# ZongyueQin/SessionSimilaritySearch

Hardware: AMD Instinct MI355X
Metric: session queries/sec (higher is better)
Workload: dtype f32

## Files before the change

### sessionsimilaritysearch_amd/csrc/scan.hip

```cpp
#include "scan_kernel.h"

namespace sss {

__device__ unsigned g_boot_expired;

extern "C" int sss_scan_boot_expired(int reset) {
    unsigned v = 0, zero = 0;
    if (hipMemcpyFromSymbol(&v, HIP_SYMBOL(g_boot_expired), sizeof(v)) != hipSuccess) { set_error("scan_boot_expired: read failed"); return SSS_EHIP; }
    if (reset && hipMemcpyToSymbol(HIP_SYMBOL(g_boot_expired), &zero, sizeof(zero)) != hipSuccess) { set_error("scan_boot_expired: reset failed"); return SSS_EHIP; }
    return (int)(v > 0x7fffffffu ? 0x7fffffffu : v);
}

int current_device() {
    int dev = 0;
    (void)hipGetDevice(&dev);
    return dev < 0 || dev >= MAX_DEVICES ? 0 : dev;
}

static int pick_splits(long n, int G, int tr) {
    int S = (256 / G) & ~7;
    if (S < 8) S = 8;
    while (S > 8 && (long)S * tr > n) S -= 8;
    return S;
}

constexpr int TR256_MIN_TILES = 24;

static size_t align256(size_t v) { return (v + 255) & ~(size_t)255; }

static ScanPlan make_plan_for(long nq, long n, int d, int k, int dtype, bool want_append);

static bool append_form_fits() {
    static int cached[MAX_DEVICES] = {};
    const int dev = current_device();
    if (cached[dev] == 0) {
        constexpr int lds = 2 * 128 * 256 + 8 * 2048;
        const void* fn = reinterpret_cast<const void*>(&k_scan<256, 128, DT_F16, 8, false, true>);
        int blocks = 0, cus = 0;
        bool ok = hipFuncSetAttribute(fn, hipFuncAttributeMaxDynamicSharedMemorySize, lds) == hipSuccess &&
                  hipOccupancyMaxActiveBlocksPerMultiprocessor(&blocks, fn, 512, lds) == hipSuccess &&
                  hipDeviceGetAttribute(&cus, hipDeviceAttributeMultiprocessorCount, dev) == hipSuccess;
        (void)hipGetLastError();
        cached[dev] = (ok && blocks >= 2 && cus >= 256) ? 1 : 2;
    }
    return cached[dev] == 1;
}

ScanPlan make_plan(long nq, long n, int d, int k, int dtype) {
    const int rb = d * elem_bytes(dtype);
    if (rb == 256 && dtype != DT_F32 && k <= KP && append_form_fits()) {
        const ScanPlan a = make_plan_for(nq, n, d, k, dtype, true);
        if (a.append) return a;
    }
    return make_plan_for(nq, n, d, k, dtype, false);
}
static ScanPlan make_plan_for(long nq, long n, int d, int k, int dtype, bool want_append) {
    ScanPlan p;
    const int rb = d * elem_bytes(dtype);
    const int wgq = rb == 1024 ? 128 : WG_QUERIES;
    p.G = (int)((nq + wgq - 1) / wgq);
    int tr = rb <= 512 ? 128 : 64;
    int S = pick_splits(n, p.G, tr);
    if (rb == 512 && (n + (long)S * 128 - 1) / ((long)S * 128) < 48) { tr = 64; S = pick_splits(n, p.G, tr); }
    if (rb == 256 && dtype != DT_F32 && n / ((long)S * 256) >= TR256_MIN_TILES) tr = 256;
    if (want_append) {
        tr = 128;
        S = pick_splits(n, p.G, tr);
        if ((long)S * p.G > 256 || (long)2 * S * tr * 7 > n) want_append = false;
        else S *= 2;
        if (!want_append) { ScanPlan none; none.append = 0; return none; }
    }
    p.tile_rows = tr;
    p.S = S;
    p.L = 2 * S;
    p.K2 = k + 2 <= KP ? (k + 2 < 8 ? 8 : k + 2) : k <= KP ? KP : k + 12;
    if ((long)p.L * KP < p.K2) p.K2 = p.L * KP;
    p.total_tiles = (int)((n + tr - 1) / tr);
    p.tiles_per_split = (p.total_tiles + S - 1) / S;
    p.cap = p.L * KP;
    const int active_splits = (p.total_tiles + p.tiles_per_split - 1) / p.tiles_per_split;
    p.J = p.K2 <= 128 ? 16 : 64;
    p.cert = 1;
    while (p.J * p.cert < p.K2 && p.cert < KP) p.cert *= 2;
    p.Ju = p.J;
    p.tau_skip = (p.cert == 1 && p.J == 16) ? 16 - p.K2 : 0;
    bool classes_ok = 2 * active_splits >= p.Ju;
    if (p.cert == 1 && p.J == 16 && active_splits < 16) {
        const int zero0 = active_splits < 8 ? 8 - active_splits : 0, zero1 = active_splits < 8 ? 8 : 16 - active_splits;
        classes_ok = zero0 <= (p.tau_skip >> 1) + (p.tau_skip & 1) && zero1 <= (p.tau_skip >> 1);
    }
    if (p.J * p.cert < p.K2 || !classes_ok) { p.J = 0; p.Ju = 0; p.tau_skip = 0; }
    p.boot = (p.J > 0 && p.cert == 1) ? 1 : 0;
    p.append = (want_append && p.boot) ? 1 : 0;
    if (want_append && !p.append) return p;
    if (p.append) p.cap = 2048;
    p.total_bytes = align256((size_t)nq * p.cap * 8);
    return p;
}

ScanPlan make_thr_plan(long nsel, long n, int d, int scan_dtype, int cap) {
    ScanPlan p = {};
    const int rb = d * elem_bytes(scan_dtype);
    const int wgq = rb == 1024 ? 128 : WG_QUERIES;
    p.G = (int)((nsel + wgq - 1) / wgq);
    p.tile_rows = rb <= 512 ? 128 : 64;
    p.S = pick_splits(n, p.G, p.tile_rows);
    p.L = 2 * p.S;
    p.total_tiles = (int)((n + p.tile_rows - 1) / p.tile_rows);
    p.tiles_per_split = (p.total_tiles + p.S - 1) / p.S;
    p.cap = cap;
    p.total_bytes = align256((size_t)nsel * cap * 8);
    return p;
}

int launch_scan(int dtype, int d, int tile_rows, const ScanArgs& a, hipStream_t st) {
    const int rb = d * elem_bytes(dtype);
    if (a.bias != nullptr) return launch_scan_l2(dtype, d, tile_rows, a, st);
    int rc = 1;
    with_dtype<true>(dtype, [&](auto dt) {
        constexpr int DT = decltype(dt)::value;
        rc = launch_shape<DT, 0>(rb, tile_rows, a, st);
    });
    if (rc != 1) return rc;
    set_error("scan: unsupported row size %d bytes", rb);
    return SSS_EINVAL;
}

}
```

### sessionsimilaritysearch_amd/csrc/scan_kernel.h

```cpp
#pragma once
#include "scan.h"
#include "scan_dev.h"

#ifndef SSS_STAGGER
#define SSS_STAGGER 1
#endif
#ifndef SSS_F32_SCHED
#define SSS_F32_SCHED 7
#endif

namespace sss {

extern __device__ unsigned g_boot_expired;

template <int RB, int TR, int DT, int NW, bool THR = false, bool AP = false, int MET = 0>
__global__ __launch_bounds__(NW * 64, AP ? 2 * (NW / 4) : NW / 4) void k_scan(const ScanArgs A) {
    constexpr int H = TR / 64;
    constexpr int CH = RB / 16;
    constexpr int NU = RB / 32;
    constexpr int TILE_BYTES = TR * RB;
    constexpr int LOADS_PER_WAVE = TR * CH / 64 / NW;
    constexpr int WGQ = NW * 32;
    constexpr bool PRECOMP = RB <= 512 && !AP;
    constexpr int TAU_LDS = 2 * TILE_BYTES;
    constexpr bool F32S = (SSS_F32_SCHED & 1) && DT == DT_F32 && !AP && !THR && RB == 512;
    static_assert(CH <= 64, "row longer than one LDS-DMA instruction");
    static_assert(LOADS_PER_WAVE >= 1, "a tile is at least one DMA piece per wave");
    extern __shared__ __attribute__((aligned(16))) char smem[];

    const int nq = A.nq, n = A.n, S = A.S, G = A.G, J = A.J;
    const char* __restrict__ Qb = reinterpret_cast<const char*>(A.Q);
    const char* __restrict__ Cb = reinterpret_cast<const char*>(A.C);
    const int tid = threadIdx.x;
    const int lane = tid & 63;
    const int wave = __builtin_amdgcn_readfirstlane(tid >> 6);
    const int r = lane & 31, h = lane >> 5;

    const int bid = blockIdx.x;
    const int xcd = bid & 7, slot = bid >> 3;
    const int split = xcd * (S >> 3) + slot / G;
    const int g = slot % G;

    const int q_local = wave * 32 + r;
    const int q_glob = g * WGQ + q_local;
    int q_ld = q_glob < nq ? q_glob : nq - 1;
    if constexpr (THR) q_ld = A.qsel[q_ld];
    f32x4 qc[NU];

    float ls[KP];
    int li[KP];
#pragma unroll
    for (int i = 0; i < KP; ++i) { ls[i] = -INFINITY; li[i] = -1; }
    float pend_s = -INFINITY;
    int pend_i = -1;
    constexpr int E = 4;
    float es[E];
    int ei[E];
    int ecnt = 0;
#pragma unroll
    for (int i = 0; i < E; ++i) { es[i] = -INFINITY; ei[i] = -1; }
    float tau = -INFINITY, thr = -INFINITY;
    if constexpr (THR) thr = q_glob < nq ? A.thr[q_glob] : INFINITY;
    float rmax = -INFINITY;
    float pub = -INFINITY;

    int tile_lo = split * A.tiles_per_split;
    int tile_hi = tile_lo + A.tiles_per_split;
    if (tile_hi > A.total_tiles) tile_hi = A.total_tiles;
    const int ntiles = tile_lo < tile_hi ? tile_hi - tile_lo : 0;
    const bool use_tau = !THR && J > 0;
    const bool boot = use_tau && A.boot && ntiles > 0;
    const int nb = boot ? 1 : 0;
    const int niter = ntiles + nb;
    auto tile_of = [&](int i) { return i < ntiles ? tile_lo + i : tile_lo; };
    const int skip = A.tau_skip;

    bool slots_seen = false;
    const unsigned* my_half = nullptr;
    unsigned cls_live = 0;
#ifdef SSS_EXP_NOPAIR
    const bool pair_pub = false;
#else
    const bool pair_pub = A.cert == 1;
#endif
    if (use_tau) {
        cls_live = pair_pub ? (unsigned)(split + (split >> 4)) & 15u : (unsigned)(2 * split + h) % (unsigned)A.Ju;
        my_half = A.slots + (size_t)q_ld * SLOT_STRIDE + h * (J >> 1);
    }
    auto tau_ord = [&]() -> unsigned {
        if (J == 16 && skip > 0) {
            unsigned v[8];
            load8_sc1(my_half, v);
            return tau_select16(v, skip, h);
        }
        unsigned m = 0xFFFFFFFFu;
        for (int v = 0; v < (J >> 1); v += 8) m = min(m, min8_sc1(my_half + v));
        return min(m, (unsigned)__shfl_xor((int)m, 32));
    };
    const unsigned tau_lds = (unsigned)(unsigned long)(lptr_c)smem + TAU_LDS + wave * 2048;
    auto tau_fetch = [&]() {
        int ln = lane;
        asm volatile("" : "+v"(ln));
#pragma unroll
        for (int j = 0; j < 2; ++j) {
            int qi = g * WGQ + wave * 32 + 16 * j + (ln >> 2);
            if (qi > nq - 1) qi = nq - 1;
            const unsigned off = (unsigned)qi * (unsigned)(SLOT_STRIDE * 4) + (unsigned)(ln & 3) * 16u;
            const unsigned dst = __builtin_amdgcn_readfirstlane(tau_lds + j * 1024);
            asm volatile("s_mov_b32 m0, %1\n\ts_nop 0\n\tglobal_load_lds_dwordx4 %0, %2 sc1"
                         : : "v"(off), "s"(dst), "s"(A.slots) : "memory");
        }
    };
    auto tau_read = [&]() -> unsigned {
        const u32x4* p = reinterpret_cast<const u32x4*>(smem + TAU_LDS + wave * 2048 + r * 64 + h * 32);
        const u32x4 a = p[0], b = p[1];
        if (skip > 0) {
            unsigned v[8] = {a.x, a.y, a.z, a.w, b.x, b.y, b.z, b.w};
            return tau_select16(v, skip, h);
        }
        const unsigned m = min(min(min(a.x, a.y), min(a.z, a.w)), min(min(b.x, b.y), min(b.z, b.w)));
        return min(m, (unsigned)__shfl_xor((int)m, 32));
    };
    auto set_tau = [&](unsigned m) {
        if (m > ORD_NEG_INF) tau = fmaxf(tau, ord2f(m - 1));
        thr = AP ? tau : fmaxf(ls[KP - 1], tau);
    };
    auto publish = [&](unsigned cls) {
        float val = rmax;
        bool ok = true;
        if (A.cert > 1) {
            float v2 = ls[1], v4 = ls[3], v8 = ls[7], v16 = ls[KP - 1];
            int i2 = li[1], i4 = li[3], i8 = li[7], i16 = li[KP - 1];
            asm volatile("" : "+v"(v2), "+v"(v4), "+v"(v8), "+v"(v16), "+v"(i2), "+v"(i4), "+v"(i8), "+v"(i16));
            const int c = A.cert;
            val = c == 2 ? v2 : c == 4 ? v4 : c == 8 ? v8 : v16;
            ok = (c == 2 ? i2 : c == 4 ? i4 : c == 8 ? i8 : i16) >= 0;
        }
        if (pair_pub) { val = fmaxf(val, __shfl_xor(val, 32)); ok = h == 0; }
        unsigned cur = 0u;
        if (J == 16 && slots_seen) cur = *reinterpret_cast<const unsigned*>(smem + TAU_LDS + wave * 2048 + r * 64 + cls * 4u);
        if (ok && val > pub && val > tau && f2ord(val) > cur && q_glob < nq) {
            int qq = THR ? q_ld : q_glob;
            asm volatile("" : "+v"(qq));
            __hip_atomic_fetch_max(A.slots + ((size_t)(unsigned)qq * (unsigned)SLOT_STRIDE + cls), f2ord(val), __ATOMIC_RELAXED, __HIP_MEMORY_SCOPE_AGENT);
            pub = val;
        }
    };

    const unsigned lds_base = (unsigned)(unsigned long)(lptr_c)smem;
    auto slot_row = [&](int i) { return ((wave * LOADS_PER_WAVE + i) * 64 + lane) / CH; };
    auto slot_off = [&](int i) {
        const int p = (wave * LOADS_PER_WAVE + i) * 64 + lane;
        const int tr = p / CH, sc = p % CH;
        return (unsigned)(tr * RB + ((sc ^ (tr & 15)) * 16));
    };
    unsigned lane_off[PRECOMP ? LOADS_PER_WAVE : 1];
    if (PRECOMP) {
#pragma unroll
        for (int i = 0; i < LOADS_PER_WAVE; ++i) lane_off[i] = slot_off(i);
    }
    auto stage_piece = [&](int buf, int tile_idx, int i) {
        const long row0 = (long)tile_idx * TR;
        const bool inside = row0 + TR <= (long)n;
        const char* tile_src = Cb + (size_t)row0 * RB;
        const unsigned dst = __builtin_amdgcn_readfirstlane(
            lds_base + buf * TILE_BYTES + (wave * LOADS_PER_WAVE + i) * 1024);
        unsigned off = PRECOMP ? lane_off[PRECOMP ? i : 0] : slot_off(i);
        if (!inside) {
            const int lr = slot_row(i);
            long grow = row0 + lr;
            if (grow > (long)n - 1) grow = (long)n - 1;
            off = (unsigned)((grow - row0) * RB) + (off - (unsigned)(lr * RB));
        }
        asm volatile("s_mov_b32 m0, %1\n\ts_nop 0\n\tglobal_load_lds_dwordx4 %0, %2"
                     : : "v"(off), "s"(dst), "s"(tile_src) : "memory");
    };
    auto stage = [&](int buf, int tile_idx) {
#pragma unroll
        for (int i = 0; i < LOADS_PER_WAVE; ++i) stage_piece(buf, tile_idx, i);
    };

    const int x = h ^ (r & 15);
    f32x16 acc0 = {0}, acc1 = {0};
    [[maybe_unused]] float bcur[MET ? 2 * H : 1];
    [[maybe_unused]] float bscale = 1.f;
    [[maybe_unused]] auto bias_fetch = [&](int tile_idx) {
#pragma unroll
        for (int s = 0; s < 2 * H; ++s) {
            long row = (long)tile_idx * TR + s * 32 + r;
            if (row > (long)n - 1) row = (long)n - 1;
            bcur[s] = h == 0 ? A.bias[row] : 0.f;
        }
    };
    [[maybe_unused]] auto bias_land = [&]() {
#pragma unroll
        for (int s = 0; s < 2 * H; ++s) asm volatile("" : "+v"(bcur[s]));
    };

    auto mfma_sub = [&](int buf, int sub, int next_tile) {
        const char* tile = smem + buf * TILE_BYTES + sub * (64 * RB);
        if constexpr (H == 1) { if (next_tile >= 0) stage(buf ^ 1, next_tile); }
        auto lda = [&](int u) -> const f32x4* {
            const int c = (2 * u) ^ x;
            return reinterpret_cast<const f32x4*>(tile + (r * CH + c) * 16);
        };
        constexpr int PF = DT == DT_F32 ? 1 : AP ? 1 : (RB == 256 ? NU : RB == 512 ? 4 : 2);
        f32x4 as0[NU], as1[NU];
#pragma unroll
        for (int u = 0; u < PF && u < NU; ++u) { const f32x4* p = lda(u); as0[u] = p[0]; as1[u] = p[32 * CH]; }
        const f32x16 zero = {0};
        if constexpr (MET) {
            float b0 = bcur[0], b1 = bcur[1];
#pragma unroll
            for (int s = 1; s < H; ++s) { b0 = sub == s ? bcur[2 * s] : b0; b1 = sub == s ? bcur[2 * s + 1] : b1; }
            acc0 = __builtin_amdgcn_mfma_f32_32x32x2f32(b0, bscale, zero, 0, 0, 0);
            acc1 = __builtin_amdgcn_mfma_f32_32x32x2f32(b1, bscale, zero, 0, 0, 0);
        } else {
            acc0 = zero; acc1 = zero;
        }
        [[maybe_unused]] i32x16 ia0 = {0}, ia1 = {0};
#pragma unroll
        for (int u = 0; u < NU; ++u) {
            if (u + PF < NU) { const f32x4* p = lda(u + PF); as0[u + PF] = p[0]; as1[u + PF] = p[32 * CH]; }
            const f32x4 a0 = as0[u], a1 = as1[u];
            __builtin_amdgcn_sched_barrier(0);
            if constexpr (DT == DT_F32) {
                acc0 = __builtin_amdgcn_mfma_f32_32x32x2f32(a0.x, qc[u].x, acc0, 0, 0, 0);
                acc1 = __builtin_amdgcn_mfma_f32_32x32x2f32(a1.x, qc[u].x, acc1, 0, 0, 0);
                acc0 = __builtin_amdgcn_mfma_f32_32x32x2f32(a0.y, qc[u].y, acc0, 0, 0, 0);
                acc1 = __builtin_amdgcn_mfma_f32_32x32x2f32(a1.y, qc[u].y, acc1, 0, 0, 0);
                acc0 = __builtin_amdgcn_mfma_f32_32x32x2f32(a0.z, qc[u].z, acc0, 0, 0, 0);
                acc1 = __builtin_amdgcn_mfma_f32_32x32x2f32(a1.z, qc[u].z, acc1, 0, 0, 0);
                acc0 = __builtin_amdgcn_mfma_f32_32x32x2f32(a0.w, qc[u].w, acc0, 0, 0, 0);
                acc1 = __builtin_amdgcn_mfma_f32_32x32x2f32(a1.w, qc[u].w, acc1, 0, 0, 0);
            } else if constexpr (DT == DT_BF16) {
                const bf16x8 qb = __builtin_bit_cast(bf16x8, qc[u]);
                acc0 = __builtin_amdgcn_mfma_f32_32x32x16_bf16(__builtin_bit_cast(bf16x8, a0), qb, acc0, 0, 0, 0);
                acc1 = __builtin_amdgcn_mfma_f32_32x32x16_bf16(__builtin_bit_cast(bf16x8, a1), qb, acc1, 0, 0, 0);
            } else if constexpr (DT == DT_F16 || DT == DT_H16) {
                const f16x8 qb = __builtin_bit_cast(f16x8, qc[u]);
                acc0 = __builtin_amdgcn_mfma_f32_32x32x16_f16(__builtin_bit_cast(f16x8, a0), qb, acc0, 0, 0, 0);
                acc1 = __builtin_amdgcn_mfma_f32_32x32x16_f16(__builtin_bit_cast(f16x8, a1), qb, acc1, 0, 0, 0);
            } else if constexpr (DT == DT_I8) {
                const i32x4 qb = __builtin_bit_cast(i32x4, qc[u]);
                ia0 = __builtin_amdgcn_mfma_i32_32x32x32_i8(__builtin_bit_cast(i32x4, a0), qb, ia0, 0, 0, 0);
                ia1 = __builtin_amdgcn_mfma_i32_32x32x32_i8(__builtin_bit_cast(i32x4, a1), qb, ia1, 0, 0, 0);
            } else {
                const bf16x8 A0 = __builtin_bit_cast(bf16x8, a0), A1 = __builtin_bit_cast(bf16x8, a1);
                const bf16x8 qh = __builtin_bit_cast(bf16x8, qc[u < NU / 2 ? u : u - NU / 2]);
                acc0 = __builtin_amdgcn_mfma_f32_32x32x16_bf16(A0, qh, acc0, 0, 0, 0);
                acc1 = __builtin_amdgcn_mfma_f32_32x32x16_bf16(A1, qh, acc1, 0, 0, 0);
                if (u < NU / 2) {
                    const bf16x8 ql = __builtin_bit_cast(bf16x8, qc[u + NU / 2]);
                    acc0 = __builtin_amdgcn_mfma_f32_32x32x16_bf16(A0, ql, acc0, 0, 0, 0);
                    acc1 = __builtin_amdgcn_mfma_f32_32x32x16_bf16(A1, ql, acc1, 0, 0, 0);
                }
            }
            __builtin_amdgcn_sched_barrier(0);
        }
        if constexpr (DT == DT_I8) {
            acc0 = __builtin_convertvector(ia0, f32x16);
            acc1 = __builtin_convertvector(ia1, f32x16);
        }
        if constexpr (H > 1) { if (sub == 0 && next_tile >= 0) stage(buf ^ 1, next_tile); }
    };

    auto block_max = [&](const f32x16& a, float& q0, float& q1, float& q2, float& q3) {
        q0 = fmaxf(fmaxf(a[0], a[1]), fmaxf(a[2], a[3]));
        q1 = fmaxf(fmaxf(a[4], a[5]), fmaxf(a[6], a[7]));
        q2 = fmaxf(fmaxf(a[8], a[9]), fmaxf(a[10], a[11]));
        q3 = fmaxf(fmaxf(a[12], a[13]), fmaxf(a[14], a[15]));
        return fmaxf(fmaxf(q0, q1), fmaxf(q2, q3));
    };
    auto insert_block = [&](const f32x16& a, int base) {
        float q0, q1, q2, q3;
        const float m = block_max(a, q0, q1, q2, q3);
        if (__builtin_amdgcn_ballot_w64(m > thr) == 0) return;
        auto walk = [&](float qm, int j0) {
            if (__builtin_amdgcn_ballot_w64(qm > thr) == 0) return;
#pragma unroll
            for (int jj = 0; jj < 4; ++jj) {
                const int j = j0 + jj;
                const bool pass = a[j] > thr;
                if (__builtin_amdgcn_ballot_w64(pass) != 0) {
                    if (__builtin_amdgcn_ballot_w64(pass && pend_i >= 0) != 0) {
                        list_insert<KP>(ls, li, pend_s, pend_i);
                        pend_s = -INFINITY; pend_i = -1;
                        thr = fmaxf(ls[KP - 1], tau);
                    }
                    const bool still = a[j] > thr;
                    pend_s = still ? a[j] : pend_s;
                    pend_i = still ? base + (j & 3) + 8 * (j >> 2) : pend_i;
                }
            }
        };
        walk(q0, 0); walk(q1, 4); walk(q2, 8); walk(q3, 12);
    };
    auto flush = [&](bool need) {
        if (need && q_glob < nq) {
            const unsigned at = atomicAdd(A.cnt + q_glob, (unsigned)ecnt);
            unsigned long long* dst = A.cand + (size_t)q_glob * A.cap;
            unsigned long long lost = 0ull;
#pragma unroll
            for (int i = 0; i < E; ++i) {
                if (i < ecnt) {
                    const unsigned long long key = make_key(es[i], ei[i]);
                    if (at + (unsigned)i < (unsigned)A.cap) dst[at + i] = key;
                    else lost = lost > key ? lost : key;
                }
            }
            if (lost != 0ull && A.maxlast != nullptr) atomicMax(A.maxlast + q_glob, lost);
        }
        ecnt = need ? 0 : ecnt;
    };
    auto append_block = [&](const f32x16& a, int base) {
        float q0, q1, q2, q3;
        const float m = block_max(a, q0, q1, q2, q3);
        if (__builtin_amdgcn_ballot_w64(m > thr) == 0) return;
        auto walk = [&](float qm, int j0) {
            if (__builtin_amdgcn_ballot_w64(qm > thr) == 0) return;
#pragma unroll
            for (int jj = 0; jj < 4; ++jj) {
                const int j = j0 + jj;
                const bool pass = a[j] > thr;
                if (__builtin_amdgcn_ballot_w64(pass) != 0) {
                    const bool full = pass && ecnt == E;
                    if (__builtin_amdgcn_ballot_w64(full) != 0) flush(full);
#pragma unroll
                    for (int i = E - 1; i > 0; --i) { es[i] = pass ? es[i - 1] : es[i]; ei[i] = pass ? ei[i - 1] : ei[i]; }
                    es[0] = pass ? a[j] : es[0];
                    ei[0] = pass ? base + (j & 3) + 8 * (j >> 2) : ei[0];
                    ecnt += pass ? 1 : 0;
                }
            }
        };
        walk(q0, 0); walk(q1, 4); walk(q2, 8); walk(q3, 12);
    };
    auto emit_block = [&](const f32x16& a, int base) {
        float q0, q1, q2, q3;
        const float m = block_max(a, q0, q1, q2, q3);
        if (__builtin_amdgcn_ballot_w64(m > thr) == 0) return;
#pragma unroll
        for (int j = 0; j < 16; ++j) {
            if (a[j] > thr) {
                const unsigned pos = atomicAdd(A.cnt + q_glob, 1u);
                if (pos < (unsigned)A.cap) A.cand[(size_t)q_glob * A.cap + pos] = make_key(a[j], base + (j & 3) + 8 * (j >> 2));
            }
        }
    };
    const bool two_ahead = H > 1 && niter > 1;
    if (ntiles > 0) stage(0, tile_lo);
    if (two_ahead) stage(1, tile_of(1));
    if constexpr (MET) {
        int q_shift = 0;
        load_queries<RB, DT>(Qb, q_ld, h, qc, &q_shift);
        if constexpr (DT == DT_F16) {
            const int e = A.corpus_shift + q_shift;
            bscale = ldexpf(1.f, e < -126 ? -126 : e > 127 ? 127 : e);
        }
        bias_fetch(tile_of(0));
    } else {
        load_queries<RB, DT>(Qb, q_ld, h, qc);
    }
    asm volatile("s_waitcnt vmcnt(0)" ::: "memory");
    __syncthreads();
    if constexpr (MET) bias_land();

    const int T = niter * H;
    long row0_of_step = 0;
    constexpr bool TAU_EVERY_TILE = TR >= 512;
    auto refresh_at = [&](int i) {
        if (i == 1 && boot && !TAU_EVERY_TILE) return false;
        if (TAU_EVERY_TILE || i <= 4) return true;
        const int sh = 30 - __builtin_clz(i);
        return (i & ((1 << sh) - 1)) == 0;
    };
    auto tile_top = [&](int i) {
        if (!use_tau || i == 0) return;
        if (J == 16) {
            if (!refresh_at(i)) return;
            publish(cls_live);
            tau_fetch();
            return;
        }
        const int ii = i - (wave >= 4 ? 1 : 0);
        if (ii >= 2 && (ii <= 8 || (ii & (ii - 1)) == 0 || (ii & 15) == 0)) set_tau(tau_ord());
        publish(cls_live);
    };
    auto tile_end = [&](int i) {
        const bool pre = boot && i == 0;
        if (pre) publish(cls_live);
        if constexpr (MET) { if (i + 1 < niter) bias_fetch(tile_of(i + 1)); }
        asm volatile("s_waitcnt vmcnt(0)" ::: "memory");
        if (use_tau && J == 16 && i > 0 && refresh_at(i)) { set_tau(tau_read()); slots_seen = true; }
        __syncthreads();
        if (pre) {
            unsigned m = 0;
            for (int it = 0; it < (AP ? 1024 : 24); ++it) {
                m = tau_ord();
                if (__builtin_amdgcn_ballot_w64(m == 0) == 0) break;
                __builtin_amdgcn_s_sleep(16);
            }
            if constexpr (!MET) {
                if (lane == 0 && __builtin_amdgcn_ballot_w64(m == 0 && q_glob < nq) != 0) atomicAdd(&g_boot_expired, 1u);
            }
            set_tau(m);
        }
        if constexpr (MET) bias_land();
    };
    auto score_mfma = [&](int t) {
        const int i = (int)((unsigned)t / (unsigned)H), sub = (int)((unsigned)t % (unsigned)H);
        if (sub == 0) tile_top(i);
        const int next_tile = (i + 1 < niter && !(two_ahead && i == 0)) ? tile_of(i + 1) : -1;
        mfma_sub(i & 1, sub, next_tile);
        row0_of_step = (long)tile_of(i) * TR + sub * 64;
        if (row0_of_step + 64 > n) {
#pragma unroll
            for (int j = 0; j < 16; ++j) {
                const int rr = (int)row0_of_step + 4 * h + (j & 3) + 8 * (j >> 2);
                if (rr >= n) acc0[j] = -INFINITY;
                if (rr + 32 >= n) acc1[j] = -INFINITY;
            }
        }
    };
    auto score_tree = [&]() -> float {
        float m0 = vmax3(acc0[0], acc0[1], acc0[2]), m1 = vmax3(acc1[0], acc1[1], acc1[2]);
#pragma unroll
        for (int j = 3; j < 15; j += 2) { m0 = vmax3(m0, acc0[j], acc0[j + 1]); m1 = vmax3(m1, acc1[j], acc1[j + 1]); }
        const float m = vmax3(m0, m1, acc0[15]);
        const float mm = vmax3(m, acc1[15], rmax);
        rmax = mm;
        return vmax3(m, acc1[15], acc1[15]);
    };
    const int t_live = nb * H;
    const bool defer = SSS_STAGGER && NW == 8 && (DT == DT_SPLIT || DT == DT_BF16 || DT == DT_H16 || DT == DT_I8) && wave >= 4;
    int t = 0;
    if constexpr (AP || THR) {
        t = T;
        for (int i = 0; i < niter; ++i) {
            tile_top(i);
            const int tile = tile_of(i);
            const int next_tile = (i + 1 < niter && !(two_ahead && i == 0)) ? tile_of(i + 1) : -1;
            const int row_base = tile * TR;
            const bool ragged = row_base + TR > n;
            const bool live = i >= nb;
            if constexpr (THR) {
                if (g * WGQ + wave * 32 >= nq) {
                    if (next_tile >= 0) stage((i & 1) ^ 1, next_tile);
                    tile_end(i);
                    continue;
                }
            }
#pragma unroll
            for (int sub = 0; sub < H; ++sub) {
                mfma_sub(i & 1, sub, next_tile);
                const int row0 = row_base + sub * 64;
                if (ragged) {
#pragma unroll
                    for (int j = 0; j < 16; ++j) {
                        const int rr = row0 + 4 * h + (j & 3) + 8 * (j >> 2);
                        if (rr >= n) acc0[j] = -INFINITY;
                        if (rr + 32 >= n) acc1[j] = -INFINITY;
                    }
                }
                const float m = score_tree();
                if (live && __builtin_amdgcn_ballot_w64(m > thr) != 0) {
                    append_block(acc0, row0 + 4 * h);
                    append_block(acc1, row0 + 32 + 4 * h);
                }
            }
            tile_end(i);
        }
    }
    if constexpr (F32S) {
        constexpr bool SPREAD = (SSS_F32_SCHED & 2) != 0, EARLY_TREE = (SSS_F32_SCHED & 4) != 0;
        static_assert(LOADS_PER_WAVE + 1 < NU, "a DMA piece per k-group, behind k-groups 1 .. LOADS_PER_WAVE");
        const unsigned frag_lane = (unsigned)(r * CH) * 16u;
        f32x4 nf0 = {0}, nf1 = {0};
        auto frag_ptr = [&](unsigned step_off, int u) -> const f32x4* {
            const int c = (2 * u) ^ x;
            return reinterpret_cast<const f32x4*>(smem + step_off + frag_lane + c * 16);
        };
        auto read_first = [&](unsigned step_off) { const f32x4* p = frag_ptr(step_off, 0); nf0 = p[0]; nf1 = p[32 * CH]; };
        float tm0 = -INFINITY;
        auto step = [&](int t) -> float {
            const int i = (int)((unsigned)t / (unsigned)H), sub = (int)((unsigned)t % (unsigned)H);
            const unsigned off = (unsigned)((i & 1) * TILE_BYTES + sub * (64 * RB));
            f32x4 as0[NU], as1[NU];
            as0[0] = nf0; as1[0] = nf1;
            const f32x16 zero = {0};
            if constexpr (MET) {
                float b0 = bcur[0], b1 = bcur[1];
#pragma unroll
                for (int s = 1; s < H; ++s) { b0 = sub == s ? bcur[2 * s] : b0; b1 = sub == s ? bcur[2 * s + 1] : b1; }
                acc0 = __builtin_amdgcn_mfma_f32_32x32x2f32(b0, bscale, zero, 0, 0, 0);
                acc1 = __builtin_amdgcn_mfma_f32_32x32x2f32(b1, bscale, zero, 0, 0, 0);
            } else {
                acc0 = zero; acc1 = zero;
            }
            auto fetch = [&](int u) { const f32x4* p = frag_ptr(off, u); as0[u] = p[0]; as1[u] = p[32 * CH]; };
            auto mfma8 = [&](int u) {
                const f32x4 a0 = as0[u], a1 = as1[u];
                __builtin_amdgcn_sched_barrier(0);
                acc0 = __builtin_amdgcn_mfma_f32_32x32x2f32(a0.x, qc[u].x, acc0, 0, 0, 0);
                acc1 = __builtin_amdgcn_mfma_f32_32x32x2f32(a1.x, qc[u].x, acc1, 0, 0, 0);
                acc0 = __builtin_amdgcn_mfma_f32_32x32x2f32(a0.y, qc[u].y, acc0, 0, 0, 0);
                acc1 = __builtin_amdgcn_mfma_f32_32x32x2f32(a1.y, qc[u].y, acc1, 0, 0, 0);
                acc0 = __builtin_amdgcn_mfma_f32_32x32x2f32(a0.z, qc[u].z, acc0, 0, 0, 0);
                acc1 = __builtin_amdgcn_mfma_f32_32x32x2f32(a1.z, qc[u].z, acc1, 0, 0, 0);
                acc0 = __builtin_amdgcn_mfma_f32_32x32x2f32(a0.w, qc[u].w, acc0, 0, 0, 0);
                acc1 = __builtin_amdgcn_mfma_f32_32x32x2f32(a1.w, qc[u].w, acc1, 0, 0, 0);
                __builtin_amdgcn_sched_barrier(0);
            };
            fetch(1);
            mfma8(0);
            if (sub == 0) tile_top(i);
            const int next_tile = (sub == 0 && i + 1 < niter && !(two_ahead && i == 0)) ? tile_of(i + 1) : -1;
            const long nrow0 = (long)next_tile * TR;
            const bool dma_plain = next_tile >= 0 && nrow0 + TR <= (long)n;
            const char* dma_src = Cb + (size_t)nrow0 * RB;
            const unsigned dma_dst = __builtin_amdgcn_readfirstlane(lds_base + ((i & 1) ^ 1) * TILE_BYTES + wave * LOADS_PER_WAVE * 1024);
            row0_of_step = (long)tile_of(i) * TR + sub * 64;
            const bool ragged_step = row0_of_step + 64 > n;
            const bool ends_tile = sub == H - 1 && !(boot && i == 0);
            if (next_tile >= 0 && (!dma_plain || !SPREAD)) stage((i & 1) ^ 1, next_tile);
#pragma unroll
            for (int u = 1; u < NU - 1; ++u) {
                fetch(u + 1);
                mfma8(u);
                if constexpr (SPREAD) {
                    if (u <= LOADS_PER_WAVE && dma_plain)
                        asm volatile("s_mov_b32 m0, %1\n\ts_nop 0\n\tglobal_load_lds_dwordx4 %0, %2"
                                     : : "v"(lane_off[u - 1]), "s"(dma_dst + (u - 1) * 1024), "s"(dma_src) : "memory");
                }
            }
            constexpr int u = NU - 1;
            if (ends_tile) {
                asm volatile("" : "+v"(as0[u]), "+v"(as1[u]));
                tile_end(i);
            }
            if (t + 1 < T && (sub < H - 1 || ends_tile))
                read_first(sub == H - 1 ? (unsigned)(((i + 1) & 1) * TILE_BYTES) : off + 64 * RB);
            if constexpr (!EARLY_TREE) {
                mfma8(u);
            } else {
                const f32x4 a0 = as0[u], a1 = as1[u];
                __builtin_amdgcn_sched_barrier(0);
                acc0 = __builtin_amdgcn_mfma_f32_32x32x2f32(a0.x, qc[u].x, acc0, 0, 0, 0);
                acc0 = __builtin_amdgcn_mfma_f32_32x32x2f32(a0.y, qc[u].y, acc0, 0, 0, 0);
                acc0 = __builtin_amdgcn_mfma_f32_32x32x2f32(a0.z, qc[u].z, acc0, 0, 0, 0);
                acc0 = __builtin_amdgcn_mfma_f32_32x32x2f32(a0.w, qc[u].w, acc0, 0, 0, 0);
                __builtin_amdgcn_sched_barrier(0);
                acc1 = __builtin_amdgcn_mfma_f32_32x32x2f32(a1.x, qc[u].x, acc1, 0, 0, 0);
                acc1 = __builtin_amdgcn_mfma_f32_32x32x2f32(a1.y, qc[u].y, acc1, 0, 0, 0);
                __builtin_amdgcn_sched_barrier(0);
                if (ragged_step) {
#pragma unroll
                    for (int j = 0; j < 16; ++j)
                        if ((int)row0_of_step + 4 * h + (j & 3) + 8 * (j >> 2) >= n) acc0[j] = -INFINITY;
                }
                tm0 = vmax3(acc0[0], acc0[1], acc0[2]);
#pragma unroll
                for (int j = 3; j < 15; j += 2) tm0 = vmax3(tm0, acc0[j], acc0[j + 1]);
                __builtin_amdgcn_sched_barrier(0);
                acc1 = __builtin_amdgcn_mfma_f32_32x32x2f32(a1.z, qc[u].z, acc1, 0, 0, 0);
                acc1 = __builtin_amdgcn_mfma_f32_32x32x2f32(a1.w, qc[u].w, acc1, 0, 0, 0);
                __builtin_amdgcn_sched_barrier(0);
            }
            if (ragged_step) {
#pragma unroll
                for (int j = 0; j < 16; ++j) {
                    const int rr = (int)row0_of_step + 4 * h + (j & 3) + 8 * (j >> 2);
                    if (!EARLY_TREE && rr >= n) acc0[j] = -INFINITY;
                    if (rr + 32 >= n) acc1[j] = -INFINITY;
                }
            }
            if constexpr (!EARLY_TREE) return score_tree();
            float m1 = vmax3_settled(acc1[0], acc1[1], acc1[2]);
#pragma unroll
            for (int j = 3; j < 15; j += 2) m1 = vmax3(m1, acc1[j], acc1[j + 1]);
            const float m = vmax3(tm0, m1, acc0[15]);
            rmax = vmax3(m, acc1[15], rmax);
            return vmax3(m, acc1[15], acc1[15]);
        };
        if (T > 0) read_first(0);
        while (t < T) {
            bool rare = false;
            for (; t < T; ++t) {
                const float m = step(t);
                if (t < t_live) {
                    if (t == t_live - 1) {
                        tile_end(0);
                        if (t + 1 < T) read_first((unsigned)TILE_BYTES);
                    }
                    continue;
                }
                if (__builtin_amdgcn_ballot_w64(m > thr) != 0) { rare = true; break; }
            }
            if (!rare) break;
            insert_block(acc0, (int)row0_of_step + 4 * h);
            insert_block(acc1, (int)row0_of_step + 32 + 4 * h);
            ++t;
        }
    }
    while (!F32S && t < T) {
        bool rare = false;
        for (; t < T; ++t) {
            const bool last = (unsigned)t % (unsigned)H == H - 1;
            const bool early = defer && t >= t_live;
            score_mfma(t);
            if (early && last) tile_end((int)((unsigned)t / (unsigned)H));
            const float m = score_tree();
            if (t >= t_live && __builtin_amdgcn_ballot_w64(m > thr) != 0) { rare = true; break; }
            if (!early && last) tile_end((int)((unsigned)t / (unsigned)H));
        }
        if (!rare) break;
        if constexpr (THR) {
            emit_block(acc0, (int)row0_of_step + 4 * h);
            emit_block(acc1, (int)row0_of_step + 32 + 4 * h);
        } else if constexpr (AP) {
            append_block(acc0, (int)row0_of_step + 4 * h);
            append_block(acc1, (int)row0_of_step + 32 + 4 * h);
        } else {
            insert_block(acc0, (int)row0_of_step + 4 * h);
            insert_block(acc1, (int)row0_of_step + 32 + 4 * h);
        }
        if (!defer && (unsigned)t % (unsigned)H == H - 1) tile_end((int)((unsigned)t / (unsigned)H));
        ++t;
    }
    if constexpr (THR) { flush(ecnt > 0); return; }
    if constexpr (AP) flush(ecnt > 0);
    list_insert<KP>(ls, li, pend_s, pend_i);
    if (!AP && q_glob < nq) {
        int nreal = 0;
#pragma unroll
        for (int i = 0; i < KP; ++i) nreal += li[i] >= 0 ? 1 : 0;
        if (nreal > 0) {
            const unsigned base = atomicAdd(A.cnt + q_glob, (unsigned)nreal);
            unsigned long long* dst = A.cand + (size_t)q_glob * A.cap + base;
#pragma unroll
            for (int i = 0; i < KP; ++i)
                if (i < nreal) dst[i] = make_key(ls[i], li[i]);
            if (nreal == KP) atomicMax(A.maxlast + q_glob, (unsigned long long)make_key(ls[KP - 1], li[KP - 1]));
        }
    }
}

template <int RB, int TR, int DT, int NW, int MET, bool THR, bool AP = false>
static int launch_form(const ScanArgs& a, hipStream_t st) {
    const size_t lds = 2 * (size_t)TR * RB + NW * 2048;
    const int rc = opt_in_lds(reinterpret_cast<const void*>(&k_scan<RB, TR, DT, NW, THR, AP, MET>), "k_scan", lds);
    if (rc) return rc;
    hipLaunchKernelGGL((k_scan<RB, TR, DT, NW, THR, AP, MET>), dim3(a.S * a.G), dim3(NW * 64), lds, st, a);
    return check_launch("k_scan");
}
template <int RB, int TR, int DT, int NW, int MET>
static int launch_one(const ScanArgs& a, hipStream_t st) {
    if (a.thr != nullptr) {
        if constexpr (TR == (RB <= 512 ? 128 : 64)) return launch_form<RB, TR, DT, NW, MET, true>(a, st);
        set_error("scan: threshold form not built for %d-row tiles of %d-byte rows", TR, RB);
        return SSS_EINVAL;
    }
    if (a.append) {
        if constexpr (RB == 256 && TR == 128 && DT != DT_F32) return launch_form<RB, TR, DT, NW, MET, false, true>(a, st);
        set_error("scan: append form not built for this shape");
        return SSS_EINVAL;
    }
    return launch_form<RB, TR, DT, NW, MET, false>(a, st);
}
template <int DT, int MET>
static int launch_shape(int rb, int tile_rows, const ScanArgs& a, hipStream_t st) {
    if (rb == 256) return tile_rows == 256 ? launch_one<256, 256, DT, 8, MET>(a, st) : launch_one<256, 128, DT, 8, MET>(a, st);
    if (rb == 512) return tile_rows == 128 ? launch_one<512, 128, DT, 8, MET>(a, st) : launch_one<512, 64, DT, 8, MET>(a, st);
    if (rb == 1024) return launch_one<1024, 64, DT, 4, MET>(a, st);
    return 1;
}

}
```

Baseline: 500,400.

## Support multi-tile bootstrap for f32 scan with cached per-step maxima to skip rescoring

Generalizes the f32 512-byte scan's bootstrap phase from one tile to a configurable number of tiles (default 1, runtime-settable up to a small maximum). Per-step score maxima from the bootstrap tiles are stored in extra LDS. At the end, revisited boot tiles are checked against the threshold via those cached maxima and skipped without rescoring when nothing can qualify. The aim is to establish a tighter threshold earlier while avoiding the rescoring cost of boot tiles. It adds LDS use and control-flow complexity, and the default of one tile changes only the skip logic.

```diff
diff --git a/sessionsimilaritysearch_amd/csrc/scan.hip b/sessionsimilaritysearch_amd/csrc/scan.hip
--- a/sessionsimilaritysearch_amd/csrc/scan.hip
+++ b/sessionsimilaritysearch_amd/csrc/scan.hip
@@ -1,3 +1,5 @@
+#include <atomic>
+
 #include "scan_kernel.h"
 
 namespace sss {
@@ -9,6 +11,12 @@
     if (hipMemcpyFromSymbol(&v, HIP_SYMBOL(g_boot_expired), sizeof(v)) != hipSuccess) { set_error("scan_boot_expired: read failed"); return SSS_EHIP; }
     if (reset && hipMemcpyToSymbol(HIP_SYMBOL(g_boot_expired), &zero, sizeof(zero)) != hipSuccess) { set_error("scan_boot_expired: reset failed"); return SSS_EHIP; }
     return (int)(v > 0x7fffffffu ? 0x7fffffffu : v);
+}
+
+constexpr int F32_BOOT_TILES = 1;
+static std::atomic<int> g_boot_tiles{0};
+extern "C" int sss_scan_boot_tiles(int tiles) {
+    return g_boot_tiles.exchange(tiles < 0 ? 0 : tiles, std::memory_order_relaxed);
 }
 
 int current_device() {
@@ -91,6 +99,12 @@
     }
     if (p.J * p.cert < p.K2 || !classes_ok) { p.J = 0; p.Ju = 0; p.tau_skip = 0; }
     p.boot = (p.J > 0 && p.cert == 1) ? 1 : 0;
+    if (p.boot && dtype == DT_F32 && rb == 512) {
+        const int want = g_boot_tiles.load(std::memory_order_relaxed);
+        p.boot = want > 0 ? want : F32_BOOT_TILES;
+        if (p.boot > BOOT_MAX) p.boot = BOOT_MAX;
+        if (p.boot > p.tiles_per_split) p.boot = p.tiles_per_split;
+    }
     p.append = (want_append && p.boot) ? 1 : 0;
     if (want_append && !p.append) return p;
     if (p.append) p.cap = 2048;
diff --git a/sessionsimilaritysearch_amd/csrc/scan_kernel.h b/sessionsimilaritysearch_amd/csrc/scan_kernel.h
--- a/sessionsimilaritysearch_amd/csrc/scan_kernel.h
+++ b/sessionsimilaritysearch_amd/csrc/scan_kernel.h
@@ -10,6 +10,10 @@
 #endif
 
 namespace sss {
+
+template <int RB, int DT, bool THR, bool AP>
+constexpr bool F32_OWN_LOOP = (SSS_F32_SCHED & 1) && DT == DT_F32 && !AP && !THR && RB == 512;
+constexpr int BOOT_MAX = 4;
 
 extern __device__ unsigned g_boot_expired;
 
@@ -23,7 +27,8 @@
     constexpr int WGQ = NW * 32;
     constexpr bool PRECOMP = RB <= 512 && !AP;
     constexpr int TAU_LDS = 2 * TILE_BYTES;
-    constexpr bool F32S = (SSS_F32_SCHED & 1) && DT == DT_F32 && !AP && !THR && RB == 512;
+    constexpr bool F32S = F32_OWN_LOOP<RB, DT, THR, AP>;
+    constexpr int BOOT_LDS = TAU_LDS + NW * 2048;
     static_assert(CH <= 64, "row longer than one LDS-DMA instruction");
     static_assert(LOADS_PER_WAVE >= 1, "a tile is at least one DMA piece per wave");
     extern __shared__ __attribute__((aligned(16))) char smem[];
@@ -70,9 +75,23 @@
     const int ntiles = tile_lo < tile_hi ? tile_hi - tile_lo : 0;
     const bool use_tau = !THR && J > 0;
     const bool boot = use_tau && A.boot && ntiles > 0;
-    const int nb = boot ? 1 : 0;
+    int nb = boot ? 1 : 0;
+    if constexpr (F32S) {
+        if (boot) { nb = A.boot < BOOT_MAX ? A.boot : BOOT_MAX; nb = nb < ntiles ? nb : ntiles; }
+    }
     const int niter = ntiles + nb;
-    auto tile_of = [&](int i) { return i < ntiles ? tile_lo + i : tile_lo; };
+    auto tile_of = [&](int i) {
+        if constexpr (F32S) return i < ntiles ? tile_lo + i : tile_lo + (i - ntiles);
+        else return i < ntiles ? tile_lo + i : tile_lo;
+    };
+    auto boot_tile = [&](int i) {
+        if constexpr (F32S) return i < nb;
+        else return boot && i == 0;
+    };
+    auto boot_last = [&](int i) {
+        if constexpr (F32S) return i == nb - 1;
+        else return true;
+    };
     const int skip = A.tau_skip;
 
     bool slots_seen = false;
@@ -370,7 +389,8 @@
     long row0_of_step = 0;
     constexpr bool TAU_EVERY_TILE = TR >= 512;
     auto refresh_at = [&](int i) {
-        if (i == 1 && boot && !TAU_EVERY_TILE) return false;
+        if constexpr (F32S) { if (i <= nb) return false; }
+        else if (i == 1 && boot && !TAU_EVERY_TILE) return false;
         if (TAU_EVERY_TILE || i <= 4) return true;
         const int sh = 30 - __builtin_clz(i);
         return (i & ((1 << sh) - 1)) == 0;
@@ -388,13 +408,13 @@
         publish(cls_live);
     };
     auto tile_end = [&](int i) {
-        const bool pre = boot && i == 0;
+        const bool pre = boot_tile(i);
         if (pre) publish(cls_live);
         if constexpr (MET) { if (i + 1 < niter) bias_fetch(tile_of(i + 1)); }
         asm volatile("s_waitcnt vmcnt(0)" ::: "memory");
         if (use_tau && J == 16 && i > 0 && refresh_at(i)) { set_tau(tau_read()); slots_seen = true; }
         __syncthreads();
-        if (pre) {
+        if (pre && boot_last(i)) {
             unsigned m = 0;
             for (int it = 0; it < (AP ? 1024 : 24); ++it) {
                 m = tau_ord();
@@ -522,7 +542,7 @@
             const unsigned dma_dst = __builtin_amdgcn_readfirstlane(lds_base + ((i & 1) ^ 1) * TILE_BYTES + wave * LOADS_PER_WAVE * 1024);
             row0_of_step = (long)tile_of(i) * TR + sub * 64;
             const bool ragged_step = row0_of_step + 64 > n;
-            const bool ends_tile = sub == H - 1 && !(boot && i == 0);
+            const bool ends_tile = sub == H - 1 && t >= t_live;
             if (next_tile >= 0 && (!dma_plain || !SPREAD)) stage((i & 1) ^ 1, next_tile);
 #pragma unroll
             for (int u = 1; u < NU - 1; ++u) {
@@ -583,24 +603,50 @@
             rmax = vmax3(m, acc1[15], rmax);
             return vmax3(m, acc1[15], acc1[15]);
         };
+        auto boot_max = [&](int s) -> float* {
+            int th = tid;
+            asm volatile("" : "+v"(th));
+            return reinterpret_cast<float*>(smem + BOOT_LDS) + s * (NW * 64) + th;
+        };
+        auto pass_step = [&](int t) {
+            const int i = (int)((unsigned)t / (unsigned)H), sub = (int)((unsigned)t % (unsigned)H);
+            if (sub == 0) {
+                tile_top(i);
+                if (i + 1 < niter) stage((i & 1) ^ 1, tile_of(i + 1));
+            }
+            if (sub == H - 1) {
+                asm volatile("" : "+v"(nf0), "+v"(nf1));
+                tile_end(i);
+            }
+            if (t + 1 < T)
+                read_first(sub == H - 1 ? (unsigned)(((i + 1) & 1) * TILE_BYTES) : (unsigned)((i & 1) * TILE_BYTES + (sub + 1) * (64 * RB)));
+        };
         if (T > 0) read_first(0);
+        int t_stop = T - t_live;
         while (t < T) {
             bool rare = false;
-            for (; t < T; ++t) {
+            for (; t < t_stop; ++t) {
                 const float m = step(t);
                 if (t < t_live) {
-                    if (t == t_live - 1) {
-                        tile_end(0);
-                        if (t + 1 < T) read_first((unsigned)TILE_BYTES);
+                    *boot_max(t) = m;
+                    if ((unsigned)t % (unsigned)H == H - 1) {
+                        const int i = (int)((unsigned)t / (unsigned)H);
+                        tile_end(i);
+                        if (t + 1 < T) read_first((unsigned)(((i + 1) & 1) * TILE_BYTES));
                     }
                     continue;
                 }
                 if (__builtin_amdgcn_ballot_w64(m > thr) != 0) { rare = true; break; }
             }
-            if (!rare) break;
-            insert_block(acc0, (int)row0_of_step + 4 * h);
-            insert_block(acc1, (int)row0_of_step + 32 + 4 * h);
-            ++t;
+            if (rare) {
+                insert_block(acc0, (int)row0_of_step + 4 * h);
+                insert_block(acc1, (int)row0_of_step + 32 + 4 * h);
+                ++t;
+            }
+            if (t < t_stop || t >= T) continue;
+            const float seen = *boot_max(t - (T - t_live));
+            if (__builtin_amdgcn_ballot_w64(seen > thr) == 0) { pass_step(t); t_stop = ++t; }
+            else t_stop = t + 1;
         }
     }
     while (!F32S && t < T) {
@@ -648,8 +694,10 @@
 
 template <int RB, int TR, int DT, int NW, int MET, bool THR, bool AP = false>
 static int launch_form(const ScanArgs& a, hipStream_t st) {
-    const size_t lds = 2 * (size_t)TR * RB + NW * 2048;
-    const int rc = opt_in_lds(reinterpret_cast<const void*>(&k_scan<RB, TR, DT, NW, THR, AP, MET>), "k_scan", lds);
+    constexpr size_t base = 2 * (size_t)TR * RB + NW * 2048, per_tile = F32_OWN_LOOP<RB, DT, THR, AP> ? (TR / 64) * NW * 256 : 0;
+    const int nboot = a.boot < 0 ? 0 : a.boot < BOOT_MAX ? a.boot : BOOT_MAX;
+    const size_t lds = base + nboot * per_tile;
+    const int rc = opt_in_lds(reinterpret_cast<const void*>(&k_scan<RB, TR, DT, NW, THR, AP, MET>), "k_scan", base + BOOT_MAX * per_tile);
     if (rc) return rc;
     hipLaunchKernelGGL((k_scan<RB, TR, DT, NW, THR, AP, MET>), dim3(a.S * a.G), dim3(NW * 64), lds, st, a);
     return check_launch("k_scan");
```

Result: no change. 501,900 (median of 6 runs) (+0.3%).
